# smn-ailab/PyCMF

Hardware: AMD Instinct MI355X
Metric: factor-update iterations/s (mu solver: one full update_step per iteration) (higher is better)
Workload: dtype f32

## Files before the change

### include/cmfhip.h

```cpp
#ifndef CMFHIP_H
#define CMFHIP_H

#include <stdint.h>

#ifdef __cplusplus
extern "C" {
#endif

typedef struct cmf_ctx cmf_ctx;

enum {
    CMF_OK = 0,
    CMF_EINVAL = 1,
    CMF_EHIP = 2,
    CMF_ENOMEM = 3,
    CMF_ENODEV = 4,
    CMF_EUNSUPPORTED = 5,
    CMF_ERCCL = 6
};

enum { CMF_U = 0, CMF_V = 1, CMF_Z = 2 };
enum { CMF_LINK_LINEAR = 0, CMF_LINK_LOGIT = 1 };
enum { CMF_UPD_U = 1, CMF_UPD_V = 2, CMF_UPD_Z = 4 };
enum { CMF_NN_U = 1, CMF_NN_V = 2, CMF_NN_Z = 4 };
// ... 63 lines not shown
int cmf_set_weight_f64(cmf_ctx *ctx, int which, const double *ptr, int64_t rs, int64_t cs);
int cmf_set_weight_f32(cmf_ctx *ctx, int which, const float *ptr, int64_t rs, int64_t cs);
int cmf_set_weighted_csr(cmf_ctx *ctx, int which, const int64_t *indptr, const int32_t *indices, const double *t_values, const double *w_values);
int cmf_clear_weight(cmf_ctx *ctx, int which);
int cmf_mu_weighted_step(cmf_ctx *ctx, double l1, double l2, int update_mask);
int cmf_weighted_residual_sq(cmf_ctx *ctx, double *ex, double *ey);
int cmf_mu_weighted_layout(cmf_ctx *ctx, int64_t *out4);
int cmf_fill_weight_synthetic(cmf_ctx *ctx, int which, uint64_t seed, double density);
int cmf_get_weight_block_f32(cmf_ctx *ctx, int which, int64_t row0, int64_t nrows, int64_t col0, int64_t ncols, float *host_dst);

int cmf_hals_step(cmf_ctx *ctx, double l1, double l2, int update_mask);
int cmf_hals_sweep(cmf_ctx *ctx, int which, const double *N, const double *G, double l1, double l2);

int cmf_als_step(cmf_ctx *ctx, double l2, int nn_mask, int update_mask);
int cmf_als_normal(cmf_ctx *ctx, int which, int64_t row0, int64_t nrows, double l2, float *host_H, float *host_g);
int cmf_als_layout(cmf_ctx *ctx, int64_t *out4);
int cmf_als_nnls_step(cmf_ctx *ctx, double l2, int nn_mask, int update_mask, int sweeps);
int cmf_als_nnls_rows(cmf_ctx *ctx, int64_t nrows, const float *host_H, const float *host_g, float *host_f, int sweeps);
int cmf_als_cg_step(cmf_ctx *ctx, double l2, int nn_mask, int update_mask, int cg_steps, int nn_sweeps);
int cmf_als_cg_rows(cmf_ctx *ctx, int which, int64_t row0, int64_t nrows, double l2, int cg_steps, float *host_f);
int cmf_als_cg_last(cmf_ctx *ctx, int64_t *out2);

int cmf_als_nncg_step(cmf_ctx *ctx, double l2, int nn_mask, int update_mask, int cg_steps, int nn_cg_steps, int nn_sweeps);
int cmf_als_nncg_rows(cmf_ctx *ctx, int which, int64_t row0, int64_t nrows, double l2, int nn_cg_steps, float *host_f);
int cmf_als_nncg_last(cmf_ctx *ctx, int64_t *out2);
int cmf_als_nncg_passes(cmf_ctx *ctx, int64_t *out2);

int cmf_als_dual_step(cmf_ctx *ctx, double l2, int nn_mask, int update_mask, int dual_max, int nn_sweeps, int nn_cg_steps);
int cmf_als_dual_rows(cmf_ctx *ctx, int which, int64_t row0, int64_t nrows, double l2, int dual_max, float *host_f);
int cmf_als_dual_last(cmf_ctx *ctx, int64_t *out5);

int cmf_set_background_weight(cmf_ctx *ctx, int which, double c0);
int cmf_get_background_weight(cmf_ctx *ctx, int which, double *c0);
int cmf_als_residual_sq(cmf_ctx *ctx, double *ex, double *ey);

int cmf_set_biases(cmf_ctx *ctx, int which, int enable, double mu, double lb);
int cmf_get_biases(cmf_ctx *ctx, int which, double *mu, double *lb, int *enabled);
int cmf_set_bias_f64(cmf_ctx *ctx, int which, int axis, const double *v);
int cmf_get_bias_f64(cmf_ctx *ctx, int which, int axis, double *v);
int cmf_als_bias_step(cmf_ctx *ctx, double l2, int nn_mask, int update_mask, int cg_steps, int nn_sweeps);
int cmf_als_bias_rows(cmf_ctx *ctx, int which, int axis, float *host_out);
int cmf_als_bias_targets(cmf_ctx *ctx, int which, int image, int64_t nnz, float *host_bt, float *host_bp);
int cmf_predict_pairs(cmf_ctx *ctx, int which, int link, int64_t n, const int64_t *rows, const int64_t *cols, float *out);

enum { CMF_LOSS_FROBENIUS = 0, CMF_LOSS_LOGISTIC = 1 };
int cmf_set_relation_loss(cmf_ctx *ctx, int which, int kind);
int cmf_get_relation_loss(cmf_ctx *ctx, int which, int *kind);
int cmf_als_logistic_loss(cmf_ctx *ctx, double *lx, double *ly);

int cmf_v_buf_elems(cmf_ctx *ctx, int64_t *n);
int cmf_mu_v_partials(cmf_ctx *ctx, float *dev_buf);
int cmf_data_pass_launches(cmf_ctx *ctx, int64_t *out5);
int cmf_mu_route_launches(cmf_ctx *ctx, int64_t *out8);
int cmf_mu_v_partials_rows(cmf_ctx *ctx, float *dev_buf, int64_t row0, int64_t nrows, int with_gram);
int cmf_mu_v_apply(cmf_ctx *ctx, const float *dev_buf, double l1, double l2);
int cmf_mu_uz_update(cmf_ctx *ctx, double l1, double l2, int update_mask);
int cmf_mu_blocked_layout(cmf_ctx *ctx, int world, int64_t *block_rows, int64_t *pbuf_elems);
int cmf_mu_v_partials_split(cmf_ctx *ctx, float *dev_P, float *dev_G);
int cmf_mu_v_apply_rows(cmf_ctx *ctx, const float *dev_P_rows, const float *dev_G, int64_t row0, int64_t nrows, double l1, double l2);
int cmf_mu_gram_v_rows(cmf_ctx *ctx, int64_t row0, int64_t nrows, float *dev_G2);
int cmf_mu_uz_update_gram(cmf_ctx *ctx, const float *dev_G2, double l1, double l2, int update_mask);

int cmf_newton_step(cmf_ctx *ctx, double alpha, double l1, double l2,
                    int x_link, int y_link, int nn_mask, int update_mask,
                    double hessian_pertubation, double sg_ratio,
                    const int32_t *u_idx, const int32_t *z_idx,
                    const int32_t *vx_idx, const int32_t *vy_idx);

int cmf_newton_step_device_sampled(cmf_ctx *ctx, double alpha, double l1, double l2,
                                   int x_link, int y_link, int nn_mask, int update_mask,
                                   double hessian_pertubation, double sg_ratio, uint64_t seed);

int cmf_sample_lists(cmf_ctx *ctx, int sweep, uint64_t seed, double sg_ratio, int64_t row0, int64_t nrows, int32_t *host_out);

int cmf_newton_uz_update(cmf_ctx *ctx, double alpha, double l1, double l2,
                         int nn_mask, int update_mask, double hessian_pertubation);
int cmf_newton_v_partials(cmf_ctx *ctx, double alpha, float *dev_buf);
int cmf_newton_v_apply(cmf_ctx *ctx, const float *dev_buf, double l1, double l2,
                       int nn_mask, double hessian_pertubation);

int cmf_newton_v_gram(cmf_ctx *ctx, double alpha, double *dev_gbuf);
int cmf_newton_v_products(cmf_ctx *ctx, double alpha, double l2, double hessian_pertubation,
                          const double *dev_gbuf, float *dev_pbuf);
int cmf_newton_v_finish(cmf_ctx *ctx, float *dev_pbuf, double l1, int nn_mask);

int cmf_residual_sq(cmf_ctx *ctx, int x_link, int y_link, double *ex2, double *ey2);
int cmf_data_sq(cmf_ctx *ctx, double *x2, double *y2);

#define CMF_TOPK_MAX_N 128
int cmf_topk(cmf_ctx *ctx, int query, int cand, int link, const int64_t *rows, int64_t nq, int n,
             const int64_t *excl_indptr, const int32_t *excl_indices, int32_t *idx, float *val);
int cmf_topk_queries(cmf_ctx *ctx, const double *Q, int64_t rs, int64_t cs, int64_t nq, int cand, int link, int n,
                     const int64_t *excl_indptr, const int32_t *excl_indices, int32_t *idx, float *val);
int cmf_topk_layout(cmf_ctx *ctx, int64_t nq, int cand, int n, int64_t excl_nnz, int own_queries, int64_t *out4);

int cmf_rank(cmf_ctx *ctx, int query, int cand, const int64_t *rows, int64_t nq,
             const int64_t *held_indptr, const int32_t *held_indices,
             const int64_t *excl_indptr, const int32_t *excl_indices,
             int32_t *rank, float *score, int32_t *eligible);
int cmf_rank_queries(cmf_ctx *ctx, const double *Q, int64_t rs, int64_t cs, int64_t nq, int cand,
             const int64_t *held_indptr, const int32_t *held_indices,
             const int64_t *excl_indptr, const int32_t *excl_indices,
             int32_t *rank, float *score, int32_t *eligible);
int cmf_rank_layout(cmf_ctx *ctx, int64_t nq, int cand, int64_t held_nnz, int64_t excl_nnz, int own_queries, int64_t *out4);

int cmf_safe_invert_batch(cmf_ctx *ctx, const double *H, double *out, int n, int k, double pert);
// ... 69 lines not shown
```

### pycmf_amd/_lib.py

```python
import ctypes as C
import os

import numpy as np

_HERE = os.path.dirname(os.path.abspath(__file__))
LIB_PATH = os.path.join(_HERE, "libcmfhip.so")

CMF_U, CMF_V, CMF_Z = 0, 1, 2
CMF_UPD_U, CMF_UPD_V, CMF_UPD_Z = 1, 2, 4
CMF_NN_U, CMF_NN_V, CMF_NN_Z = 1, 2, 4
LINKS = {"linear": 0, "logit": 1}
RELATION_LOSSES = {"frobenius": 0, "logistic": 1}
UPD_U, UPD_V, UPD_Z = 1, 2, 4
K_GEMM_NN, K_GEMM_TN, K_GEMM_NT, K_ELEMWISE, K_EIGEN = 0, 1, 2, 3, 4
KERNEL_CLASSES = {"gemm_nn": 0, "gemm_tn": 1, "gemm_nt": 2, "elementwise": 3, "eigen": 4, "gemm_small": 5, "spmm": 6, "rowhess": 7, "gemm_pair": 8, "topk": 9, "klmu": 10}
LATER_KERNEL_CLASSES = {"hals": 11}

_ERR = {1: ValueError, 2: RuntimeError, 3: MemoryError, 4: RuntimeError, 5: NotImplementedError}

_i64, _i32, _dbl, _vp = C.c_int64, C.c_int, C.c_double, C.c_void_p
_pd = C.POINTER(C.c_double)
_pf = C.POINTER(C.c_float)
_pi32 = C.POINTER(C.c_int32)
_pi64 = C.POINTER(C.c_int64)
# ... 26 lines not shown
    "cmf_get_factor_f64": [_vp, _i32, _pd, _i64, _i64],
    "cmf_mu_step": [_vp, _dbl, _dbl, _i32],
    "cmf_mu_step_error": [_vp, _dbl, _dbl, _i32, _pd, _pd],
    "cmf_mu_kl_step": [_vp, _dbl, _dbl, _i32],
    "cmf_kl_divergence": [_vp, _pd, _pd],
    "cmf_mu_kl_layout": [_vp, _pi64],
    "cmf_mu_beta_step": [_vp, _dbl, _dbl, _dbl, _i32],
    "cmf_beta_divergence": [_vp, _dbl, _pd, _pd],
    "cmf_mu_beta_products": [_vp, _dbl, _i32, _pf, _pf],
    "cmf_mu_beta_layout": [_vp, _pi64],
    "cmf_set_weight_f64": [_vp, _i32, _pd, _i64, _i64],
    "cmf_set_weight_f32": [_vp, _i32, _pf, _i64, _i64],
    "cmf_set_weighted_csr": [_vp, _i32, _pi64, _pi32, _pd, _pd],
    "cmf_clear_weight": [_vp, _i32],
    "cmf_mu_weighted_step": [_vp, _dbl, _dbl, _i32],
    "cmf_weighted_residual_sq": [_vp, _pd, _pd],
    "cmf_mu_weighted_layout": [_vp, _pi64],
    "cmf_fill_weight_synthetic": [_vp, _i32, C.c_uint64, _dbl],
    "cmf_get_weight_block_f32": [_vp, _i32, _i64, _i64, _i64, _i64, _pf],
    "cmf_hals_step": [_vp, _dbl, _dbl, _i32],
    "cmf_hals_sweep": [_vp, _i32, _pd, _pd, _dbl, _dbl],
    "cmf_als_step": [_vp, _dbl, _i32, _i32],
    "cmf_als_normal": [_vp, _i32, _i64, _i64, _dbl, _pf, _pf],
    "cmf_als_layout": [_vp, _pi64],
    "cmf_als_nnls_step": [_vp, _dbl, _i32, _i32, _i32],
    "cmf_als_nnls_rows": [_vp, _i64, _pf, _pf, _pf, _i32],
    "cmf_als_cg_step": [_vp, _dbl, _i32, _i32, _i32, _i32],
    "cmf_als_cg_rows": [_vp, _i32, _i64, _i64, _dbl, _i32, _pf],
    "cmf_als_cg_last": [_vp, _pi64],
    "cmf_als_nncg_step": [_vp, _dbl, _i32, _i32, _i32, _i32, _i32],
    "cmf_als_nncg_rows": [_vp, _i32, _i64, _i64, _dbl, _i32, _pf],
    "cmf_als_nncg_last": [_vp, _pi64],
    "cmf_als_nncg_passes": [_vp, _pi64],
    "cmf_als_dual_step": [_vp, _dbl, _i32, _i32, _i32, _i32, _i32],
    "cmf_als_dual_rows": [_vp, _i32, _i64, _i64, _dbl, _i32, _pf],
    "cmf_als_dual_last": [_vp, _pi64],
    "cmf_set_background_weight": [_vp, _i32, _dbl],
    "cmf_get_background_weight": [_vp, _i32, _pd],
    "cmf_als_residual_sq": [_vp, _pd, _pd],
    "cmf_set_biases": [_vp, _i32, _i32, _dbl, _dbl],
    "cmf_get_biases": [_vp, _i32, _pd, _pd, C.POINTER(C.c_int)],
    "cmf_set_bias_f64": [_vp, _i32, _i32, _pd],
    "cmf_get_bias_f64": [_vp, _i32, _i32, _pd],
    "cmf_als_bias_step": [_vp, _dbl, _i32, _i32, _i32, _i32],
    "cmf_als_bias_rows": [_vp, _i32, _i32, _pf],
    "cmf_als_bias_targets": [_vp, _i32, _i32, _i64, _pf, _pf],
    "cmf_predict_pairs": [_vp, _i32, _i32, _i64, _pi64, _pi64, _pf],
    "cmf_set_relation_loss": [_vp, _i32, _i32],
    "cmf_get_relation_loss": [_vp, _i32, C.POINTER(C.c_int)],
    "cmf_als_logistic_loss": [_vp, _pd, _pd],
    "cmf_v_buf_elems": [_vp, _pi64],
    "cmf_data_pass_launches": [_vp, _pi64],
    "cmf_mu_route_launches": [_vp, _pi64],
    "cmf_mu_v_partials": [_vp, _vp],
    "cmf_mu_v_apply": [_vp, _vp, _dbl, _dbl],
    "cmf_mu_v_partials_rows": [_vp, _vp, _i64, _i64, _i32],
    "cmf_mu_uz_update": [_vp, _dbl, _dbl, _i32],
    "cmf_mu_blocked_layout": [_vp, _i32, _pi64, _pi64],
    "cmf_mu_v_partials_split": [_vp, _vp, _vp],
    "cmf_mu_v_apply_rows": [_vp, _vp, _vp, _i64, _i64, _dbl, _dbl],
    "cmf_mu_gram_v_rows": [_vp, _i64, _i64, _vp],
    "cmf_mu_uz_update_gram": [_vp, _vp, _dbl, _dbl, _i32],
    "cmf_newton_step": [_vp, _dbl, _dbl, _dbl, _i32, _i32, _i32, _i32, _dbl, _dbl,
                        _pi32, _pi32, _pi32, _pi32],
    "cmf_newton_step_device_sampled": [_vp, _dbl, _dbl, _dbl, _i32, _i32, _i32, _i32, _dbl, _dbl, C.c_uint64],
    "cmf_newton_uz_update": [_vp, _dbl, _dbl, _dbl, _i32, _i32, _dbl],
    "cmf_newton_v_partials": [_vp, _dbl, _vp],
    "cmf_newton_v_apply": [_vp, _vp, _dbl, _dbl, _i32, _dbl],
    "cmf_newton_v_gram": [_vp, _dbl, _vp],
    "cmf_newton_v_products": [_vp, _dbl, _dbl, _dbl, _vp, _vp],
    "cmf_newton_v_finish": [_vp, _vp, _dbl, _i32],
    "cmf_residual_sq": [_vp, _i32, _i32, _pd, _pd],
    "cmf_data_sq": [_vp, _pd, _pd],
    "cmf_topk": [_vp, _i32, _i32, _i32, _pi64, _i64, _i32, _pi64, _pi32, _pi32, _pf],
    "cmf_topk_queries": [_vp, _pd, _i64, _i64, _i64, _i32, _i32, _i32, _pi64, _pi32, _pi32, _pf],
    "cmf_topk_layout": [_vp, _i64, _i32, _i32, _i64, _i32, _pi64],
    "cmf_rank": [_vp, _i32, _i32, _pi64, _i64, _pi64, _pi32, _pi64, _pi32, _pi32, _pf, _pi32],
    "cmf_rank_queries": [_vp, _pd, _i64, _i64, _i64, _i32, _pi64, _pi32, _pi64, _pi32, _pi32, _pf, _pi32],
    "cmf_rank_layout": [_vp, _i64, _i32, _i64, _i64, _i32, _pi64],
    "cmf_safe_invert_batch": [_vp, _pd, _pd, _i32, _i32, _dbl],
    "cmf_safe_invert_f64": [_vp, _pd, _pd, _i32, _dbl],
    "cmf_safe_solve_batch": [_vp, _pd, _pd, _pd, _pd, _i32, _i32, _dbl, _i32],
    "cmf_debug_clock": [_vp, _pd, _pd],
    "cmf_kernel_timing": [_vp, _i32],
    "cmf_kernel_time": [_vp, _i32, _pd, _pi64, _pd],
    "cmf_kernel_timing_reset": [_vp],
    "cmf_rowhess_samples": [_vp, _pd, _pd],
    "cmf_marker": [_vp],
    "cmf_marker_times": [_vp, _pd, _i64, _pi64],
    "cmf_get_stream": [_vp, C.POINTER(_vp)],
    "cmf_get_geometry": [_vp, _pi64, _pi64, _pi64, C.POINTER(C.c_int)],
    "cmf_factor_dev_ptr": [_vp, _i32, C.POINTER(_pf)],
    "cmf_scratch_alloc": [_vp, _i64, C.POINTER(_vp)],
    "cmf_scratch_free": [_vp, _vp],
    "cmf_export_factor_rows": [_vp, _i32, _vp],
    "cmf_import_factor_rows": [_vp, _i32, _vp],
    "cmf_comm_unique_id": [C.c_char_p],
    "cmf_comm_init": [_vp, _i32, _i32, C.c_char_p],
    "cmf_comm_destroy": [_vp],
    "cmf_comm_info": [_vp, C.POINTER(C.c_int), C.POINTER(C.c_int)],
    "cmf_comm_allreduce_f32": [_vp, _vp, _i64],
    "cmf_comm_allreduce_f64": [_vp, _vp, _i64],
    "cmf_comm_allreduce_f32_bg": [_vp, _vp, _i64],
    "cmf_comm_join": [_vp],
    "cmf_comm_exposed_ms": [_vp, _pd, _i32],
    "cmf_comm_allgather_f32": [_vp, _vp, _i64],
# ... 497 lines not shown
    def als_bias_targets(self, which, image, nnz):
        nnz = int(nnz)
        if nnz < 0:
            raise ValueError("als_bias_targets: nnz must be the number of stored entries, got %d" % nnz)
        bt, bp = np.zeros(nnz, dtype=np.float32), np.zeros(nnz, dtype=np.float32)
        check(self._lib.cmf_als_bias_targets(self._h, which, image, nnz, bt.ctypes.data_as(_pf), bp.ctypes.data_as(_pf)))
        return bt, bp

    def set_relation_loss(self, which, kind):
        check(self._lib.cmf_set_relation_loss(self._h, which, RELATION_LOSSES.get(kind, kind)))

    def get_relation_loss(self, which):
        kind = C.c_int(0)
        check(self._lib.cmf_get_relation_loss(self._h, which, C.byref(kind)))
        return kind.value

    def als_logistic_loss(self, want_x=True, want_y=True):
        lx, ly = C.c_double(0), C.c_double(0)
        check(self._lib.cmf_als_logistic_loss(self._h, C.byref(lx) if want_x else None, C.byref(ly) if want_y else None))
        return lx.value, ly.value

    def predict_pairs(self, which, rows, cols, link="linear"):
        rows = np.ascontiguousarray(rows, dtype=np.int64).ravel()
        cols = np.ascontiguousarray(cols, dtype=np.int64).ravel()
        if rows.shape != cols.shape:
            raise ValueError("predict_pairs: rows and cols must have one length, got %d and %d" % (rows.size, cols.size))
        out = np.zeros(rows.size, dtype=np.float32)
        check(self._lib.cmf_predict_pairs(self._h, which, LINKS[link] if isinstance(link, str) else int(link), rows.size,
                                          rows.ctypes.data_as(_pi64), cols.ctypes.data_as(_pi64), out.ctypes.data_as(_pf)))
        return out

    def mu_step_error(self, l1, l2, mask=7):
        ex2, ey2 = C.c_double(0), C.c_double(0)
        check(self._lib.cmf_mu_step_error(self._h, l1, l2, mask, C.byref(ex2), C.byref(ey2)))
        return ex2.value, ey2.value

    def v_buf_elems(self):
        n = C.c_int64(0)
        check(self._lib.cmf_v_buf_elems(self._h, C.byref(n)))
        return n.value

    def data_pass_launches(self):
        out = np.zeros(5, dtype=np.int64)
        check(self._lib.cmf_data_pass_launches(self._h, out.ctypes.data_as(_pi64)))
        return tuple(int(v) for v in out)

    MU_ROUTE_FORMS = ("epi_mu", "factor_update", "factor_update2", "pair", "gram32", "sum_slabs", "mu_apply", "narrow_copy")

    def mu_route_launches(self):
        out = np.zeros(8, dtype=np.int64)
        check(self._lib.cmf_mu_route_launches(self._h, out.ctypes.data_as(_pi64)))
        return dict(zip(self.MU_ROUTE_FORMS, (int(v) for v in out)))

    def mu_v_partials(self, dev_ptr):
        check(self._lib.cmf_mu_v_partials(self._h, _vp(dev_ptr)))

    def mu_v_partials_rows(self, dev_ptr, row0, nrows, with_gram):
        check(self._lib.cmf_mu_v_partials_rows(self._h, _vp(dev_ptr), row0, nrows, 1 if with_gram else 0))

    def mu_v_apply(self, dev_ptr, l1, l2):
        check(self._lib.cmf_mu_v_apply(self._h, _vp(dev_ptr), l1, l2))

    def mu_uz_update(self, l1, l2, mask=7):
        check(self._lib.cmf_mu_uz_update(self._h, l1, l2, mask))

    def mu_blocked_layout(self, world):
        b, n = C.c_int64(0), C.c_int64(0)
        check(self._lib.cmf_mu_blocked_layout(self._h, int(world), C.byref(b), C.byref(n)))
        return b.value, n.value

    def mu_v_partials_split(self, dev_p, dev_g):
        check(self._lib.cmf_mu_v_partials_split(self._h, _vp(dev_p), _vp(dev_g)))

    def mu_v_apply_rows(self, dev_p_rows, dev_g, row0, nrows, l1, l2):
        check(self._lib.cmf_mu_v_apply_rows(self._h, _vp(dev_p_rows), _vp(dev_g), row0, nrows, l1, l2))

    def mu_gram_v_rows(self, row0, nrows, dev_g2):
        check(self._lib.cmf_mu_gram_v_rows(self._h, row0, nrows, _vp(dev_g2)))

    def mu_uz_update_gram(self, dev_g2, l1, l2, mask=7):
        check(self._lib.cmf_mu_uz_update_gram(self._h, _vp(dev_g2), l1, l2, mask))

    def factor_dev_ptr(self, which):
        p = _pf()
        check(self._lib.cmf_factor_dev_ptr(self._h, which, C.byref(p)))
        return C.cast(p, _vp).value

    def run(self, solver, max_iter, tol, l1=0.0, l2=0.0, alpha=0.5, alpha_err=0.5, x_link="linear", y_link="linear", nn_mask=0,
            update_mask=7, pert=0.2, ratio=1.0, seed=0, check_every=10):
        prm = RunParams(0 if solver == "mu" else 1, l1, l2, alpha, alpha_err, LINKS[x_link], LINKS[y_link], nn_mask, update_mask,
                        pert, ratio, int(seed))
        cap = max_iter // max(check_every, 1) + 2
        errs, secs = (C.c_double * cap)(), (C.c_double * cap)()
        n_iter, n_trace = C.c_int(0), C.c_int(0)
        check(self._lib.cmf_run(self._h, C.byref(prm), int(max_iter), float(tol), int(check_every), C.byref(n_iter), errs, secs, cap,
                                C.byref(n_trace)))
        n = min(n_trace.value, cap)
        return n_iter.value, [errs[i] for i in range(n)], [secs[i] for i in range(n)]

    def newton_step(self, alpha, l1, l2, x_link, y_link, nn_mask, upd_mask, pert, ratio,
                    u_idx=None, z_idx=None, vx_idx=None, vy_idx=None):
        def ptr(a):
            if a is None:
                return None
            a = np.ascontiguousarray(a, dtype=np.int32)
            self._keep.append(a)
# ... 300 lines not shown
```

### pycmf_amd/csrc/cmf_api.hip

```cpp
#include "../../include/cmfhip.h"
#include "cmf_kernels.hip.h"
#include "cmf_gemm_wg256.hip.h"
#include "cmf_gemm_pair.hip.h"
#include "cmf_eigen.hip.h"
#include "cmf_chol_mfma.hip.h"
#include "cmf_sparse.hip.h"
#include "cmf_rowhess.hip.h"
#include "cmf_bf16x6.hip.h"
#include "cmf_rowhess6.hip.h"
#include "cmf_shared64.hip.h"
#include "cmf_refine64.hip.h"
#include "cmf_eigclamp.hip.h"
#include "cmf_rank1clamp.hip.h"

#include <hip/hip_runtime.h>

#include <algorithm>
#include <chrono>
#include <cmath>
#include <cstdarg>
#include <cstdio>
#include <cstdlib>
#include <cstring>
#include <mutex>
#include <numeric>
#include <set>
#include <string>
#include <thread>
#include <type_traits>
#include <vector>

using namespace cmfk;

static thread_local std::string g_err;

static int fail(int code, const char *fmt, ...) {
    char buf[512];
    va_list ap;
    va_start(ap, fmt);
    vsnprintf(buf, sizeof buf, fmt, ap);
    va_end(ap);
    g_err = buf;
    return code;
}

#define HIPCHK(expr)                                                                       \
    do {                                                                                   \
        hipError_t e_ = (expr);                                                            \
        if (e_ != hipSuccess)                                                              \
            return fail(e_ == hipErrorOutOfMemory ? CMF_ENOMEM : CMF_EHIP, "%s failed: %s (%s:%d)", \
                        #expr, hipGetErrorString(e_), __FILE__, __LINE__);                 \
    } while (0)
#define CHK(expr)                 \
    do {                          \
        int rc_ = (expr);         \
        if (rc_ != CMF_OK) return rc_; \
// ... 24 lines not shown
    int32_t *idx = nullptr;
    float *pv = nullptr, *wv = nullptr, *tv = nullptr;
    float *ev = nullptr;
    float *bt = nullptr, *bp = nullptr;
    int64_t rows = 0, cols = 0, nnz = 0;
};

namespace cmfk { struct AlsBiasPiece; }
struct AlsBias {
    bool on = false, dirty = false;
    double mu = 0.0, lb = 0.0;
    float *r = nullptr, *c = nullptr;
    cmfk::AlsBiasPiece *pieces[2] = {nullptr, nullptr};
    int64_t *first[2] = {nullptr, nullptr};
    int64_t npieces[2] = {0, 0};
    int64_t L = 0;
};

struct StepGraph {
    hipGraphExec_t exec = nullptr;
    double key[8] = {0};
    int warm = 0;
    bool failed = false;
};

struct EvPair {
    hipEvent_t a, b;
    int cls;
    double flops;
};

struct CmfComm;
struct cmf_ctx {
    int device = 0;
    CmfComm *comm = nullptr;
    hipStream_t stream = nullptr;
    bool own_stream = false;
    int num_cu = 256;

    int64_t m = 0, d = 0, p = 0;
    int k = 0;
    int64_t mp = 0, dp = 0, pp = 0;
    int kp = 0;
    bool have_problem = false;
    unsigned long long *dbg_stamps = nullptr;
    bool diag_ok = false;
    int opt_graph = -1;
    StepGraph mu_graph, newton_graph;
    int opt_split = -1;
    int opt_data_pass_wg = 15;
    int64_t data_pass_launches[5] = {0, 0, 0, 0, 0};
    int64_t mu_route_launches[8] = {0, 0, 0, 0, 0, 0, 0, 0};
    int opt_pair = 1;
    int opt_arith_min_tiles = 8;
    int opt_arith = 0;
    int opt_ns = 1;
    bool hess_psd = true;
    int opt_pipe_nt = 4;
    int opt_topk_split = 0;
    int opt_kl_split = 0;
    DevBuf kl_slab, kl_small, kl_part;
    int opt_beta_route = 0;
    DevBuf beta_slab, beta_small, beta_part;
    int opt_wmu_split = 0;
    int wm_kind[2] = {0, 0};
    float *wm_w[2] = {nullptr, nullptr}, *wm_p[2] = {nullptr, nullptr};
    WCsrDev wm_sp[2][2];
    DevBuf wm_slab, wm_small, wm_part;
    DevBuf hals_ws;
    int opt_als_piece = 0;
    DevBuf als_h, als_part, als_g, als_sol, als_desc;
    DevBuf als_nnls_ws;
    int opt_als_cg_lds = -1;
    DevBuf als_cg_ws;
    int opt_als_cg_piece = 0;
    DevBuf als_cg_long;
    int64_t als_cg_last[2] = {0, 0};
    int64_t als_nncg_last[4] = {0, 0, 0, 0};
    DevBuf als_nncg_passes;
    std::vector<int32_t> als_nncg_lens;
    bool als_nncg_counted = true;
    int als_dual_perm = 0;
    int64_t als_dual_last[5] = {0, 0, 0, 0, 0};
    DevBuf als_dual_ws;
    double wm_bg[2] = {0.0, 0.0};
    DevBuf als_bg_s, als_bg64;
    int rel_loss[2] = {0, 0};
    AlsBias als_bias[2];
    int opt_als_bias_piece = 0;
    DevBuf als_bias_part, als_bias_ws;
    int opt_choldiag = 0;
    int opt_chol = 1;
    int opt_chol_mfma = 1;
    int opt_zlogit_l2 = 1;
    int opt_rowdiag = 0;
    int opt_rowsym = 4;
    int opt_rowstagger = 1;
    int opt_rowkernel = 1;
    double flop_scale = 1.0;
    bool dev_sampling = false;
    uint64_t dev_seed = 0;
    int64_t sample_off[3] = {0, 0, 0};

    float *X = nullptr, *Y = nullptr;
    CsrDev sp[2][2];
    bool sparse[2] = {false, false};
// ... 640 lines not shown
        c->sparse[w] = false;
        c->sp_sq[w] = 0.0;
        for (int t = 0; t < 2; ++t) c->sp[w][t] = CsrDev();
    }
}

static void pin_give(void *p);
extern "C" int cmf_comm_destroy(cmf_ctx *c);
extern "C" int cmf_ctx_destroy(cmf_ctx *c) {
    if (!c) return CMF_OK;
    DeviceGuard dg(c->device);
    (void)cmf_comm_destroy(c);
    release_problem(c);
    for (void *p : c->scratch) (void)hipFree(p);
    c->scratch.clear();
    (void)hipFree(c->dscalar);
    for (auto &e : c->pending) { (void)hipEventDestroy(e.a); (void)hipEventDestroy(e.b); }
    for (auto e : c->evpool) (void)hipEventDestroy(e);
    for (auto e : c->markers) (void)hipEventDestroy(e);
    for (int b = 0; b < 2; ++b) {
        pin_give(c->pin[b]);
        if (c->pin_ev[b]) (void)hipEventDestroy(c->pin_ev[b]);
    }
    if (c->own_stream) (void)hipStreamDestroy(c->stream);
    delete c;
    return CMF_OK;
}

extern "C" int cmf_set_option(cmf_ctx *c, const char *name, int64_t value) {
    if (!c || !name) return fail(CMF_EINVAL, "null argument");
    invalidate_graphs(c);
    if (!strcmp(name, "graph")) {
        c->opt_graph = value < 0 ? -1 : (value != 0);
        return CMF_OK;
    }
    if (!strcmp(name, "gemm_pipe_nt")) {
        c->opt_pipe_nt = (int)value;
    } else if (!strcmp(name, "gemm_split")) {
        c->opt_split = (int)value;
    } else if (!strcmp(name, "data_pass_wg")) {
        if (value < 0 || value > 15)
            return fail(CMF_EINVAL, "data_pass_wg: bit 0 the TN data passes, bit 1 the NN data passes, bit 2 / bit 3 their factor from a register ring (0..15)");
        c->opt_data_pass_wg = (int)value;
    } else if (!strcmp(name, "small_gram_shares")) {
        c->opt_gram32_shares = (int)std::max<int64_t>(1, std::min<int64_t>(value, 1024));
    } else if (!strcmp(name, "small_gram")) {
        c->opt_gram32 = value != 0;
    } else if (!strcmp(name, "chol_mfma")) {
        c->opt_chol_mfma = value != 0;
    } else if (!strcmp(name, "narrow_update")) {
        c->opt_narrow_update = value != 0;
    } else if (!strcmp(name, "pair_passes")) {
        c->opt_pair = (int)value;
    } else if (!strcmp(name, "z_logit_hessian_l2")) {
        c->opt_zlogit_l2 = value != 0;
    } else if (!strcmp(name, "row_diag")) {
#ifndef CMF_DIAG_BUILD
        if (value != 0) return fail(CMF_EINVAL, "row_diag is a timing-only diagnostic (wrong results) that the default build does not carry: "
                                                "build with `python -m pycmf_amd.build --diag` and set CMF_DIAG=1");
#endif
        if (value != 0 && !c->diag_ok) return fail(CMF_EINVAL, "row_diag is a timing-only diagnostic (wrong results): set CMF_DIAG=1 in the environment to allow it");
        c->opt_rowdiag = (int)value;
    } else if (!strcmp(name, "row_stagger")) {
        c->opt_rowstagger = value != 0;
    } else if (!strcmp(name, "row_symmetric")) {
        c->opt_rowsym = (int)value;
    } else if (!strcmp(name, "row_kernel")) {
        c->opt_rowkernel = value != 0;
    } else if (!strcmp(name, "direct_newton_step")) {
        c->opt_direct_step = value != 0;
    } else if (!strcmp(name, "row_certificates")) {
        c->opt_rowcert = value != 0;
    } else if (!strcmp(name, "row_classes")) {
        if (value < -1 || value > 6) return fail(CMF_EINVAL, "row_classes: -1 (automatic), 0 (off) or 2..6 rows per group");
        c->opt_rowclasses = (int)value;
    } else if (!strcmp(name, "row_chunk")) {
        c->opt_rowchunk = std::max<int64_t>(0, value);
    } else if (!strcmp(name, "sample_row_offset_u")) {
        c->sample_off[CMF_U] = value;
    } else if (!strcmp(name, "sample_row_offset_v")) {
        c->sample_off[CMF_V] = value;
    } else if (!strcmp(name, "sample_row_offset_z")) {
        c->sample_off[CMF_Z] = value;
    } else if (!strcmp(name, "gemm_arith")) {
        if (value != 0 && value != 1) return fail(CMF_EINVAL, "gemm_arith must be 0 (fp32 MFMA) or 1 (bf16x6)");
        c->opt_arith = (int)value;
    } else if (!strcmp(name, "gemm_arith_min_tiles")) {
        c->opt_arith_min_tiles = (int)std::max<int64_t>(1, value);
    } else if (!strcmp(name, "trace_error")) {
        c->opt_trace_error_off = value == 0;
    } else if (!strcmp(name, "eig_clamp")) {
        c->opt_eig_clamp = (int)value;
    } else if (!strcmp(name, "rank1_clamp")) {
        c->opt_rank1_clamp = value != 0;
    } else if (!strcmp(name, "newton_schulz")) {
        c->opt_ns = value != 0;
    } else if (!strcmp(name, "chol_diag")) {
#ifndef CMF_DIAG_BUILD
        if (value != 0) return fail(CMF_EINVAL, "chol_diag is a timing-only diagnostic (wrong results) that the default build does not carry: "
                                                "build with `python -m pycmf_amd.build --diag` and set CMF_DIAG=1");
#endif
        if (value != 0 && !c->diag_ok) return fail(CMF_EINVAL, "chol_diag is a timing-only diagnostic (wrong results): set CMF_DIAG=1 in the environment to allow it");
        c->opt_choldiag = (int)value;
    } else if (!strcmp(name, "safe_inverse_cholesky")) {
        c->opt_chol = value != 0;
    } else if (!strcmp(name, "small_tile_update")) {
// ... 411 lines not shown
}

extern "C" int cmf_scratch_alloc(cmf_ctx *c, int64_t bytes, void **dev_ptr) {
    if (!c || !dev_ptr || bytes < 0) return fail(CMF_EINVAL, "bad scratch request");
    DeviceGuard dg(c->device);
    const size_t n = bytes ? (size_t)bytes : 16;
    HIPCHK(hipMalloc(dev_ptr, n));
    c->scratch.push_back(*dev_ptr);
    HIPCHK(hipMemsetAsync(*dev_ptr, 0, n, c->stream));
    return CMF_OK;
}

extern "C" int cmf_scratch_free(cmf_ctx *c, void *dev_ptr) {
    if (!c) return fail(CMF_EINVAL, "null context");
    if (!dev_ptr) return CMF_OK;
    DeviceGuard dg(c->device);
    auto it = std::find(c->scratch.begin(), c->scratch.end(), dev_ptr);
    if (it == c->scratch.end()) return fail(CMF_EINVAL, "not a scratch buffer of this context");
    HIPCHK(hipStreamSynchronize(c->stream));
    c->scratch.erase(it);
    (void)hipFree(dev_ptr);
    return CMF_OK;
}

extern "C" int cmf_export_factor_rows(cmf_ctx *c, int which, float *dev_dst) {
    NEED_PROBLEM(c);
    if (which < 0 || which > 2 || !dev_dst) return fail(CMF_EINVAL, "bad factor argument");
    DeviceGuard dg(c->device);
    HIPCHK(hipMemcpyAsync(dev_dst, c->F[which], (size_t)c->frows[which] * c->kp * sizeof(float), hipMemcpyDeviceToDevice, c->stream));
    return CMF_OK;
}

extern "C" int cmf_import_factor_rows(cmf_ctx *c, int which, const float *dev_src) {
    NEED_PROBLEM(c);
    if (which < 0 || which > 2 || !dev_src) return fail(CMF_EINVAL, "bad factor argument");
    DeviceGuard dg(c->device);
    HIPCHK(hipMemcpyAsync(c->F[which], dev_src, (size_t)c->frows[which] * c->kp * sizeof(float), hipMemcpyDeviceToDevice, c->stream));
    return CMF_OK;
}

extern "C" int cmf_v_buf_elems(cmf_ctx *c, int64_t *n) {
    NEED_PROBLEM(c);
    if (!n) return fail(CMF_EINVAL, "null argument");
    *n = c->dp * c->kp + (int64_t)c->kp * c->kp;
    return CMF_OK;
}

extern "C" int cmf_data_pass_launches(cmf_ctx *c, int64_t *out5) {
    if (!c || !out5) return fail(CMF_EINVAL, "cmf_data_pass_launches: null context or output");
    for (int f = 0; f < 5; ++f) out5[f] = c->data_pass_launches[f];
    return CMF_OK;
}

extern "C" int cmf_mu_route_launches(cmf_ctx *c, int64_t *out8) {
    if (!c || !out8) return fail(CMF_EINVAL, "cmf_mu_route_launches: null context or output");
    for (int f = 0; f < 8; ++f) out8[f] = c->mu_route_launches[f];
    return CMF_OK;
}

extern "C" int cmf_mu_v_partials(cmf_ctx *c, float *buf) {
    NEED_PROBLEM(c);
    if (!buf) return fail(CMF_EINVAL, "null buffer");
    if (!have_data(c, 0) || !have_data(c, 1)) return fail(CMF_EINVAL, "X and Y must be set before a V update");
    DeviceGuard dg(c->device);
    float *P = buf, *Gs = buf + c->dp * c->kp;
    CHK(data_times(c, 0, true, c->F[CMF_U], P));
    CHK(data_times(c, 1, false, c->F[CMF_Z], P, true));
    CHK(gram32(c, c->F[CMF_U], c->mp + c->pp, Gs));
    return CMF_OK;
}

extern "C" int cmf_mu_v_partials_rows(cmf_ctx *c, float *buf, int64_t row0, int64_t nrows, int with_gram) {
    NEED_PROBLEM(c);
    if (!buf) return fail(CMF_EINVAL, "null buffer");
    if (!c->X || !c->Y) return fail(CMF_EUNSUPPORTED, "cmf_mu_v_partials_rows needs dense images of X and Y");
    if (c->opt_arith != 0) return fail(CMF_EUNSUPPORTED, "cmf_mu_v_partials_rows: fp32 MFMA arithmetic only");
    if (row0 < 0 || nrows <= 0 || row0 % 256 || nrows % 256 || row0 + nrows > c->dp) return fail(CMF_EINVAL, "row block must be 256-aligned inside [0, d_pad)");
    DeviceGuard dg(c->device);
    float *P = buf + row0 * c->kp;
    CHK(gemm(c, MODE_TN, c->X + row0, c->dp, c->F[CMF_U], c->kp, P, nrows, c->kp, c->mp));
    CHK(gemm(c, MODE_NN, c->Y + row0 * c->pp, c->pp, c->F[CMF_Z], c->kp, P, nrows, c->kp, c->pp, true));
    if (with_gram)
        CHK(gram32(c, c->F[CMF_U], c->mp + c->pp, buf + c->dp * c->kp));
    return CMF_OK;
}

extern "C" int cmf_mu_v_apply(cmf_ctx *c, const float *buf, double l1, double l2) {
    NEED_PROBLEM(c);
    if (!buf) return fail(CMF_EINVAL, "null buffer");
    DeviceGuard dg(c->device);
    const float *P = buf, *Gs = buf + c->dp * c->kp;
    return mu_update(c, c->F[CMF_V], Gs, P, c->dp, l1, l2);
}

struct PairSide { int which; bool trans; const float *B; };
static void pair_shape(const cmf_ctx *c, const PairSide &sd, int64_t *mout, int64_t *kred) {
    const int64_t rp = sd.which == 0 ? c->mp : c->dp, cp = sd.which == 0 ? c->dp : c->pp;
    *mout = sd.trans ? cp : rp; *kred = sd.trans ? rp : cp;
}
static bool pair_ok(const cmf_ctx *c, const PairSide &a0, const PairSide &a1) {
    if (!c->opt_pair || c->kp != 128 || !c->X || !c->Y || c->opt_arith || c->opt_split > 0 || !c->opt_fused_mu || !c->opt_small_tile)
        return false;
    for (const PairSide *sd : {&a0, &a1}) {
        int64_t mout, kred;
        pair_shape(c, *sd, &mout, &kred);
        if (mout / 256 >= (int64_t)(c->num_cu * 3) / 4 || kred < 256 || !small_tile_ok(c, mout)) return false;
    }
    return true;
}
static int data_times_pair(cmf_ctx *c, const PairSide &a0, const PairSide &a1, SlabRef *s0, SlabRef *s1) {
    PairArgs g;
    memset(&g, 0, sizeof g);
    const PairSide *sides[2] = {&a0, &a1};
    SlabRef *refs[2] = {s0, s1};
    DevBuf *bufs[2] = {&c->slabs, &c->slabs_b};
    int64_t unit = 0, mout[2];
    double flops = 0.0;
    for (int i = 0; i < 2; ++i) {
        int64_t kred;
        pair_shape(c, *sides[i], &mout[i], &kred);
        PairProb &p = g.p[i];
        p.A = sides[i]->which == 0 ? c->X : c->Y; p.lda = sides[i]->which == 0 ? c->dp : c->pp;
        p.B = sides[i]->B; p.ldb = c->kp;
        p.mode = sides[i]->trans ? MODE_TN : MODE_NN;
        p.tiles = (int)(mout[i] / 256); p.ksteps = (int)(kred / 32);
        p.unit0 = unit; p.slab_stride = mout[i] * c->kp;
        unit += (int64_t)p.tiles * p.ksteps;
        flops += 2.0 * (double)mout[i] * (double)c->kp * (double)kred;
    }
    g.total = unit;
    g.quota = (unit + c->num_cu - 1) / c->num_cu;
    const int64_t nwg = (unit + g.quota - 1) / g.quota;
    for (int i = 0; i < 2; ++i) {
        PairProb &p = g.p[i];
        const int64_t maxslots = (p.ksteps + g.quota - 1) / g.quota + 1;
        CHK(ensure(c, *bufs[i], (size_t)maxslots * p.slab_stride * sizeof(float)));
        p.C = (float *)bufs[i]->p;
        refs[i]->base = p.C; refs[i]->nslab = (int)maxslots; refs[i]->stride = p.slab_stride;
        refs[i]->quota = g.quota; refs[i]->unit0 = p.unit0; refs[i]->ksteps = p.ksteps;
    }
    constexpr size_t lds = GemmCfg<MODE_NN, 128>::LDS_BYTES > GemmCfg<MODE_TN, 128>::LDS_BYTES ? GemmCfg<MODE_NN, 128>::LDS_BYTES : GemmCfg<MODE_TN, 128>::LDS_BYTES;
    CHK(allow_big_lds(c, reinterpret_cast<const void *>(&gemm_pair_kernel), (int)lds));
    Timed tm(c, CMF_K_GEMM_PAIR, flops * c->flop_scale);
    hipLaunchKernelGGL(gemm_pair_kernel, dim3((unsigned)nwg), dim3(512), lds, c->stream, g);
    ++c->mu_route_launches[3];
    HIPCHK(hipGetLastError());
    return CMF_OK;
}

static int mu_uz_update_with(cmf_ctx *c, const float *G2, double l1, double l2, int mask);
extern "C" int cmf_mu_uz_update(cmf_ctx *c, double l1, double l2, int mask) {
    NEED_PROBLEM(c);
    DeviceGuard dg(c->device);
    if (!(mask & (CMF_UPD_U | CMF_UPD_Z))) return CMF_OK;
    CHK(gram32(c, c->F[CMF_V], c->dp, c->G2));
    return mu_uz_update_with(c, c->G2, l1, l2, mask);
}

static int grow_v(cmf_ctx *c, int64_t rows) {
    if (rows <= c->v_rows_alloc) return CMF_OK;
    invalidate_graphs(c);
    float *nv = nullptr;
    CHK(dev_alloc(c, (void **)&nv, (size_t)rows * c->kp * sizeof(float)));
    HIPCHK(hipMemcpyAsync(nv, c->F[CMF_V], (size_t)c->dp * c->kp * sizeof(float), hipMemcpyDeviceToDevice, c->stream));
    HIPCHK(hipStreamSynchronize(c->stream));
    dev_free(c, c->F[CMF_V]);
    c->F[CMF_V] = nv;
    c->v_rows_alloc = rows;
    return CMF_OK;
}
extern "C" int cmf_mu_blocked_layout(cmf_ctx *c, int world, int64_t *block_rows, int64_t *pbuf_elems) {
    NEED_PROBLEM(c);
    if (world < 1) return fail(CMF_EINVAL, "world must be >= 1");
    DeviceGuard dg(c->device);
    const int64_t tiles = c->dp / 256;
    const int64_t B = 256 * ((tiles + world - 1) / world);
    CHK(grow_v(c, B * world));
    if (block_rows) *block_rows = B;
    if (pbuf_elems) *pbuf_elems = B * world * c->kp;
    return CMF_OK;
}
extern "C" int cmf_mu_v_partials_split(cmf_ctx *c, float *P, float *G) {
    NEED_PROBLEM(c);
    if (!P || !G) return fail(CMF_EINVAL, "null buffer");
    if (!have_data(c, 0) || !have_data(c, 1)) return fail(CMF_EINVAL, "X and Y must be set before a V update");
    DeviceGuard dg(c->device);
    CHK(gram32(c, c->F[CMF_U], c->mp + c->pp, G));
    CHK(data_times(c, 0, true, c->F[CMF_U], P));
    CHK(data_times(c, 1, false, c->F[CMF_Z], P, true));
    return CMF_OK;
}
extern "C" int cmf_mu_v_apply_rows(cmf_ctx *c, const float *P_rows, const float *G, int64_t row0, int64_t nrows, double l1, double l2) {
    NEED_PROBLEM(c);
    if (!P_rows || !G) return fail(CMF_EINVAL, "null buffer");
    if (row0 < 0 || nrows < 0 || row0 % 256 || nrows % 256 || row0 + nrows > c->dp) return fail(CMF_EINVAL, "row block must be 256-aligned inside [0, d_pad)");
    if (nrows == 0) return CMF_OK;
    DeviceGuard dg(c->device);
    return mu_update(c, c->F[CMF_V] + row0 * c->kp, G, P_rows, nrows, l1, l2);
// ... 333 lines not shown
```

Baseline: 17.19.

## Add 256-thread buffer-load MFMA pair GEMM kernel for data passes

Adds a new gemm_pair_wg_kernel with 256 threads per workgroup, 256x128 tiles, raw buffer loads, register prefetch of the F operand, double-buffered LDS only for the NN A operand, and explicitly scheduled MFMA 32x32x2 f32. It is enabled by default when leading dimensions fit in 32-bit offsets, replacing the 512-thread pair kernel for the V-partials data passes. The aim is higher per-wave work and better latency hiding through software pipelining. The risks are more registers per thread and lower occupancy, plus new indexing code that must stay correct.

```diff
diff --git a/include/cmfhip.h b/include/cmfhip.h
--- a/include/cmfhip.h
+++ b/include/cmfhip.h
@@ -139,6 +139,7 @@
 int cmf_mu_v_partials(cmf_ctx *ctx, float *dev_buf);
 int cmf_data_pass_launches(cmf_ctx *ctx, int64_t *out5);
 int cmf_mu_route_launches(cmf_ctx *ctx, int64_t *out8);
+int cmf_pair_pass_launches(cmf_ctx *ctx, int64_t *out2);
 int cmf_mu_v_partials_rows(cmf_ctx *ctx, float *dev_buf, int64_t row0, int64_t nrows, int with_gram);
 int cmf_mu_v_apply(cmf_ctx *ctx, const float *dev_buf, double l1, double l2);
 int cmf_mu_uz_update(cmf_ctx *ctx, double l1, double l2, int update_mask);
diff --git a/pycmf_amd/_lib.py b/pycmf_amd/_lib.py
--- a/pycmf_amd/_lib.py
+++ b/pycmf_amd/_lib.py
@@ -102,6 +102,7 @@
     "cmf_v_buf_elems": [_vp, _pi64],
     "cmf_data_pass_launches": [_vp, _pi64],
     "cmf_mu_route_launches": [_vp, _pi64],
+    "cmf_pair_pass_launches": [_vp, _pi64],
     "cmf_mu_v_partials": [_vp, _vp],
     "cmf_mu_v_apply": [_vp, _vp, _dbl, _dbl],
     "cmf_mu_v_partials_rows": [_vp, _vp, _i64, _i64, _i32],
@@ -705,6 +706,11 @@
         check(self._lib.cmf_mu_route_launches(self._h, out.ctypes.data_as(_pi64)))
         return dict(zip(self.MU_ROUTE_FORMS, (int(v) for v in out)))
 
+    def pair_pass_launches(self):
+        out = np.zeros(2, dtype=np.int64)
+        check(self._lib.cmf_pair_pass_launches(self._h, out.ctypes.data_as(_pi64)))
+        return tuple(int(v) for v in out)
+
     def mu_v_partials(self, dev_ptr):
         check(self._lib.cmf_mu_v_partials(self._h, _vp(dev_ptr)))
 
diff --git a/pycmf_amd/csrc/cmf_api.hip b/pycmf_amd/csrc/cmf_api.hip
--- a/pycmf_amd/csrc/cmf_api.hip
+++ b/pycmf_amd/csrc/cmf_api.hip
@@ -2,6 +2,7 @@
 #include "cmf_kernels.hip.h"
 #include "cmf_gemm_wg256.hip.h"
 #include "cmf_gemm_pair.hip.h"
+#include "cmf_gemm_pair_wg.hip.h"
 #include "cmf_eigen.hip.h"
 #include "cmf_chol_mfma.hip.h"
 #include "cmf_sparse.hip.h"
@@ -132,6 +133,8 @@
     int64_t data_pass_launches[5] = {0, 0, 0, 0, 0};
     int64_t mu_route_launches[8] = {0, 0, 0, 0, 0, 0, 0, 0};
     int opt_pair = 1;
+    int opt_pair_wg = 1;
+    int64_t pair_pass_launches[2] = {0, 0};
     int opt_arith_min_tiles = 8;
     int opt_arith = 0;
     int opt_ns = 1;
@@ -878,6 +881,9 @@
         c->opt_narrow_update = value != 0;
     } else if (!strcmp(name, "pair_passes")) {
         c->opt_pair = (int)value;
+    } else if (!strcmp(name, "pair_pass_wg")) {
+        if (value < 0 || value > 1) return fail(CMF_EINVAL, "pair_pass_wg: 0 (gemm_pair_kernel, 512 threads) or 1 (gemm_pair_wg_kernel, 256 threads)");
+        c->opt_pair_wg = (int)value;
     } else if (!strcmp(name, "z_logit_hessian_l2")) {
         c->opt_zlogit_l2 = value != 0;
     } else if (!strcmp(name, "row_diag")) {
@@ -1395,6 +1401,12 @@
     return CMF_OK;
 }
 
+extern "C" int cmf_pair_pass_launches(cmf_ctx *c, int64_t *out2) {
+    if (!c || !out2) return fail(CMF_EINVAL, "cmf_pair_pass_launches: null context or output");
+    for (int f = 0; f < 2; ++f) out2[f] = c->pair_pass_launches[f];
+    return CMF_OK;
+}
+
 extern "C" int cmf_mu_route_launches(cmf_ctx *c, int64_t *out8) {
     if (!c || !out8) return fail(CMF_EINVAL, "cmf_mu_route_launches: null context or output");
     for (int f = 0; f < 8; ++f) out8[f] = c->mu_route_launches[f];
@@ -1482,11 +1494,19 @@
         refs[i]->base = p.C; refs[i]->nslab = (int)maxslots; refs[i]->stride = p.slab_stride;
         refs[i]->quota = g.quota; refs[i]->unit0 = p.unit0; refs[i]->ksteps = p.ksteps;
     }
-    constexpr size_t lds = GemmCfg<MODE_NN, 128>::LDS_BYTES > GemmCfg<MODE_TN, 128>::LDS_BYTES ? GemmCfg<MODE_NN, 128>::LDS_BYTES : GemmCfg<MODE_TN, 128>::LDS_BYTES;
-    CHK(allow_big_lds(c, reinterpret_cast<const void *>(&gemm_pair_kernel), (int)lds));
-    Timed tm(c, CMF_K_GEMM_PAIR, flops * c->flop_scale);
-    hipLaunchKernelGGL(gemm_pair_kernel, dim3((unsigned)nwg), dim3(512), lds, c->stream, g);
+    const bool wg = c->opt_pair_wg && g.p[0].lda < ((int64_t)1 << 21) && g.p[1].lda < ((int64_t)1 << 21) && c->kp < ((int64_t)1 << 21);
+    if (wg) {
+        CHK(allow_big_lds(c, reinterpret_cast<const void *>(&gemm_pair_wg_kernel), (int)PairWgCfg::LDS_BYTES));
+        Timed tm(c, CMF_K_GEMM_PAIR, flops * c->flop_scale);
+        hipLaunchKernelGGL(gemm_pair_wg_kernel, dim3((unsigned)nwg), dim3(PairWgCfg::NT), PairWgCfg::LDS_BYTES, c->stream, g);
+    } else {
+        constexpr size_t lds = GemmCfg<MODE_NN, 128>::LDS_BYTES > GemmCfg<MODE_TN, 128>::LDS_BYTES ? GemmCfg<MODE_NN, 128>::LDS_BYTES : GemmCfg<MODE_TN, 128>::LDS_BYTES;
+        CHK(allow_big_lds(c, reinterpret_cast<const void *>(&gemm_pair_kernel), (int)lds));
+        Timed tm(c, CMF_K_GEMM_PAIR, flops * c->flop_scale);
+        hipLaunchKernelGGL(gemm_pair_kernel, dim3((unsigned)nwg), dim3(512), lds, c->stream, g);
+    }
     ++c->mu_route_launches[3];
+    ++c->pair_pass_launches[wg ? 1 : 0];
     HIPCHK(hipGetLastError());
     return CMF_OK;
 }
diff --git a/pycmf_amd/csrc/cmf_gemm_pair_wg.hip.h b/pycmf_amd/csrc/cmf_gemm_pair_wg.hip.h
--- /dev/null
+++ b/pycmf_amd/csrc/cmf_gemm_pair_wg.hip.h
@@ -0,0 +1,163 @@
+#pragma once
+#include "cmf_kernels.hip.h"
+#include "cmf_gemm_pair.hip.h"
+
+namespace cmfk {
+
+struct PairWgCfg {
+    static constexpr int BM = 256, BN = 128, BK = 32, PADK = BK + 4, NT = 256;
+    static constexpr int STAGE = BM * PADK;
+    static constexpr int LD = BM * BK / 4 / NT;
+    static constexpr size_t LDS_BYTES = 2 * STAGE * sizeof(float);
+};
+
+template <int MODE>
+__device__ __forceinline__ void pair_wg_segment(const PairProb &pb, const int tile, const int ks, const int len, const int slot, float *smem) {
+    using C = PairWgCfg;
+    static_assert(MODE == MODE_NN || MODE == MODE_TN, "data passes: NN and TN");
+    constexpr bool NN = (MODE == MODE_NN);
+    constexpr int NGRP = C::BK / 2;
+    constexpr int XREG_MI = 2, FREG_MI = 5;
+    const int t = threadIdx.x, lane = t & 63, wid = t >> 6;
+    const int l31 = lane & 31, lh = lane >> 5;
+    const int wrow0 = 128 * (wid >> 1), wcol0 = 64 * (wid & 1);
+    const int64_t row0 = (int64_t)tile * C::BM;
+    const int64_t kbeg = (int64_t)ks * C::BK;
+    const int64_t klast = kbeg + (int64_t)(len - 1) * C::BK;
+    const int lda = (int)pb.lda, ldb = (int)pb.ldb;
+
+    f32x16 acc[4][2];
+#pragma unroll
+    for (int i = 0; i < 4; ++i)
+#pragma unroll
+        for (int j = 0; j < 2; ++j)
+#pragma unroll
+            for (int r = 0; r < 16; ++r) acc[i][j][r] = 0.0f;
+
+    f32x4 ra[NN ? C::LD : 1];
+    f32x4 xr[NN ? 1 : NGRP];
+    f32x2 br[NGRP];
+    const char *Xu = reinterpret_cast<const char *>(NN ? pb.A + row0 * pb.lda : pb.A + row0), *Fu = reinterpret_cast<const char *>(pb.B);
+    auto rsrc = [&](const char *origin) { return __builtin_amdgcn_make_buffer_rsrc(const_cast<char *>(origin), 0, -1, 0x00020000); };
+    const uint32_t x_off = (uint32_t)(4 * (NN ? (t >> 3) * lda + 4 * (t & 7) : lh * lda + wrow0 + 4 * l31));
+    const uint32_t f_off = (uint32_t)(4 * ((NN ? 4 * lh : lh) * ldb + wcol0 + 2 * l31));
+    const int a_lds = (t >> 3) * C::PADK + 4 * (t & 7);
+
+    auto gload_xu = [&](int64_t k0, int s) {
+        xr[s] = __builtin_bit_cast(f32x4, __builtin_amdgcn_raw_buffer_load_b128(rsrc(Xu + k0 * pb.lda * 4), x_off, 2 * s * lda * 4, 0));
+    };
+    auto gload_au = [&](int64_t k0, int p) {
+        ra[p] = __builtin_bit_cast(f32x4, __builtin_amdgcn_raw_buffer_load_b128(rsrc(Xu + k0 * 4), x_off, 32 * p * lda * 4, 0));
+    };
+    auto lstore_a = [&](float *As, int p) { *reinterpret_cast<f32x4 *>(As + a_lds + 32 * p * C::PADK) = ra[p]; };
+    auto gload_f = [&](int64_t k0, int s) {
+        br[s] = __builtin_bit_cast(f32x2, __builtin_amdgcn_raw_buffer_load_b64(rsrc(Fu + k0 * pb.ldb * 4), f_off,
+                                                                                 (NN ? 8 * (s >> 2) + (s & 3) : 2 * s) * ldb * 4, 0));
+    };
+
+    if constexpr (NN) {
+        const int64_t k1 = kbeg + C::BK < klast ? kbeg + C::BK : klast;
+#pragma unroll
+        for (int p = 0; p < C::LD; ++p) gload_au(kbeg, p);
+        __builtin_amdgcn_sched_barrier(0);
+#pragma unroll
+        for (int p = 0; p < C::LD; ++p) lstore_a(smem, p);
+        __builtin_amdgcn_sched_barrier(0);
+#pragma unroll
+        for (int p = 0; p < C::LD; ++p) {
+            gload_au(k1, p);
+            __builtin_amdgcn_sched_barrier(0);
+            if (p == FREG_MI) {
+                gload_f(kbeg, 0);
+                __builtin_amdgcn_sched_barrier(0);
+            }
+        }
+#pragma unroll
+        for (int s = 1; s < NGRP - 1; ++s) {
+            gload_f(kbeg, s);
+            __builtin_amdgcn_sched_barrier(0);
+        }
+        __syncthreads();
+    } else {
+#pragma unroll
+        for (int s = 0; s < NGRP - 1; ++s) {
+            gload_xu(kbeg, s);
+            __builtin_amdgcn_sched_barrier(0);
+            gload_f(kbeg, s);
+            __builtin_amdgcn_sched_barrier(0);
+        }
+    }
+
+    int kt = 0;
+    do {
+        const float *As = smem + (kt & 1) * C::STAGE;
+        float *nAs = smem + ((kt + 1) & 1) * C::STAGE;
+        const int64_t k0 = kbeg + (int64_t)kt * C::BK;
+        int64_t kn1 = k0 + C::BK, kn2 = kn1 + C::BK;
+        kn1 = kn1 < klast ? kn1 : klast;
+        kn2 = kn2 < klast ? kn2 : klast;
+        f32x4 a[NN ? 2 : 1][4];
+        auto lda_frag = [&](int q) {
+#pragma unroll
+            for (int i = 0; i < 4; ++i)
+                a[q & 1][i] = *reinterpret_cast<const f32x4 *>(As + (wrow0 + 32 * i + l31) * C::PADK + 4 * (2 * q + lh));
+        };
+        if constexpr (NN) lda_frag(0);
+#pragma unroll
+        for (int sidx = 0; sidx < NGRP; ++sidx) {
+            const int q = sidx >> 2, e = sidx & 3;
+            if constexpr (NN)
+                if (e == 0 && q + 1 < NGRP / 4) lda_frag(q + 1);
+            __builtin_amdgcn_sched_barrier(0);
+#pragma unroll
+            for (int mi = 0; mi < 8; ++mi) {
+                const int i = mi >> 1, j = mi & 1;
+                const float av = NN ? a[NN ? q & 1 : 0][i][e] : xr[NN ? 0 : sidx][i];
+                acc[i][j] = __builtin_amdgcn_mfma_f32_32x32x2f32(av, br[sidx][j], acc[i][j], 0, 0, 0);
+                if constexpr (NN) {
+                    if (sidx == 0) lstore_a(nAs, mi);
+                    if (sidx == 1) gload_au(kn2, mi);
+                }
+                const int rs = (sidx + NGRP - 1) % NGRP;
+                const int64_t kr = sidx == 0 ? k0 : kn1;
+                if (!NN && mi == XREG_MI) gload_xu(kr, rs);
+                if (mi == FREG_MI) gload_f(kr, rs);
+                __builtin_amdgcn_sched_barrier(0);
+            }
+        }
+        if constexpr (NN) __syncthreads();
+    } while (++kt < len);
+
+    float *Cl = pb.C + (int64_t)slot * pb.slab_stride + (row0 + wrow0 + (NN ? 4 : 16) * lh) * C::BN + wcol0 + 2 * l31;
+#pragma unroll
+    for (int i = 0; i < 4; ++i) {
+#pragma unroll
+        for (int j = 0; j < 2; ++j) asm volatile("" : "+a"(acc[i][j]));
+#pragma unroll
+        for (int r = 0; r < 16; ++r) {
+            const int rr = (r & 3) + 8 * (r >> 2);
+            *reinterpret_cast<f32x2 *>(Cl + (NN ? 32 * i + rr : 4 * rr + i) * C::BN) = f32x2{acc[i][0][r], acc[i][1][r]};
+        }
+        __builtin_amdgcn_sched_barrier(0);
+    }
+}
+
+__global__ __launch_bounds__(256) void gemm_pair_wg_kernel(PairArgs g) {
+    extern __shared__ __attribute__((aligned(16))) float smem[];
+    int64_t u = (int64_t)blockIdx.x * g.quota;
+    const int64_t end = (u + g.quota < g.total) ? u + g.quota : g.total;
+    while (u < end) {
+        const int pi = (u >= g.p[1].unit0) ? 1 : 0;
+        const PairProb &pb = g.p[pi];
+        const int64_t local = u - pb.unit0;
+        const int tile = (int)(local / pb.ksteps), ks = (int)(local - (int64_t)tile * pb.ksteps);
+        const int64_t left = end - u;
+        const int len = (int)(left < pb.ksteps - ks ? left : pb.ksteps - ks);
+        const int slot = (int)((int64_t)blockIdx.x - (pb.unit0 + (int64_t)tile * pb.ksteps) / g.quota);
+        if (pb.mode == MODE_TN) pair_wg_segment<MODE_TN>(pb, tile, ks, len, slot, smem);
+        else pair_wg_segment<MODE_NN>(pb, tile, ks, len, slot, smem);
+        u += len;
+    }
+}
+
+}
```

Result: no change. 17.21, median of 3 (+0.1%).
